# microsoft/M3P

Measured on AMD Instinct MI355X. Metric: pre-train samples/sec (whole node), 12L/768d seq=128+36, higher is better.
Workload: dtype bf16; 1 GPU; cfg2: 12L/768d/12h, 36 regions + 128 tokens, V=250002, 19 MLM targets/seq + ITM BCE, dropout 0.10, adam_inverse_sqrt + clip 5; per_gpu_batch=256, global_batch=256, seq_len=164, parallelism=dp1, prewarm_steps=36

## Files before the change

include/m3p_hip.h:

```cpp
#ifndef M3P_HIP_H
#define M3P_HIP_H

#include <stddef.h>
#include <stdint.h>

#ifdef __cplusplus
extern "C" {
#endif

#define M3P_API __attribute__((visibility("default")))

#define M3P_OK 0
#define M3P_EINVAL (-1)
#define M3P_ENOTIMPL (-2)
#define M3P_ENOMEM (-3)

M3P_API const char* m3p_version(void);


enum {
  M3P_EPI_NONE = 0,
  M3P_EPI_BIAS = 1,
  M3P_EPI_BIAS_GELU = 2,
  M3P_EPI_BIAS_DROP_RES = 3,
// ... 44 lines not shown
                                    int M, int N, int K, float alpha, void* stream);
M3P_API int m3p_gemm_nn_streamk_f32(const void* A, int lda, const void* W, int ldw, int k_valid, float* C,
                                    int ldc, int M, int N, int K, float alpha, void* stream);
M3P_API int m3p_gemm_nn_w4_f32(const void* A, int lda, const void* W, int ldw, float* C, int ldc, int M, int N, int K, float alpha,
                               void* workspace, size_t workspace_bytes, void* stream);

M3P_API size_t m3p_gemm_wgrad_workspace_bytes(void);
M3P_API int m3p_gemm_wgrad_bf16(const void* dY, int lddy, const void* X, int ldx, float* dW, int lddw,
                                int M, int N, int K, float alpha, void* workspace, size_t workspace_bytes,
                                void* stream);
M3P_API int m3p_gemm_wgrad_store_bf16(const void* dY, int lddy, const void* X, int ldx, float* dW, int lddw, int M, int N, int K,
                                      float alpha, void* workspace, size_t workspace_bytes, void* stream);
M3P_API int m3p_gemm_wgrad_pair_bf16(const void* dYa, int lddya, const void* Xa, int ldxa, float* dWa, int lddwa, int Na, int Ka,
                                     const void* dYb, int lddyb, const void* Xb, int ldxb, float* dWb, int lddwb, int Nb, int Kb,
                                     int M, float alpha, void* workspace, size_t workspace_bytes, void* stream);


M3P_API int m3p_layernorm_fwd(const void* x, const float* gamma, const float* beta, const uint8_t* rowmask,
                              void* y, float* mean, float* rstd, int rows, int d, float eps, void* stream);

M3P_API int m3p_layernorm_bwd(const void* dy_a, const void* dy_b, const void* x, const float* gamma,
                              const float* mean, const float* rstd, const uint8_t* rowmask,
                              void* dx, void* dx_drop, float* dgamma, float* dbeta, float* dbias_drop,
                              int rows, int d, uint32_t seed, uint32_t thresh24, float inv_keep, void* stream);
M3P_API int m3p_layernorm_bwd_rows(const void* dy_a, const void* dy_b, const void* x, const float* gamma,
                                   const float* mean, const float* rstd, const uint8_t* rowmask,
                                   void* dx, void* dx_drop, float* dgamma, float* dbeta, float* dbias_drop,
                                   int rows, int d, uint32_t seed, uint32_t thresh24, float inv_keep,
                                   const int32_t* rng_rows, void* stream);

// ... 178 lines not shown
```

m3p_amd/csrc/gemm.hip:

```cpp
#include <mutex>
#include <type_traits>
#include "common.hpp"
#include "../../include/m3p_hip.h"
#include <hip/amd_detail/amd_hip_unsafe_atomics.h>

static int g_variant = 1;
extern "C" void m3p_debug_set_variant(int v) { g_variant = (v == 2 || v == 6) ? v : 1; }

namespace {

constexpr int BK = 64;
constexpr int ROWB = BK * 2;

template <int EPI>
__device__ __forceinline__ void epilogue_store(const M3PEpilogue& ep, bf16* __restrict__ C, int ldc,
                                               int M, int N, int m, int n, f32x4 acc, f32x4& csum) {
  if (m >= M || n >= N) return;
  const bool full = (n + 3 < N);
  float v[4] = {acc[0], acc[1], acc[2], acc[3]};
  const float alpha = (ep.alpha == 0.f) ? 1.f : ep.alpha;
  if (EPI == M3P_EPI_NONE || EPI == M3P_EPI_BIAS || EPI == M3P_EPI_RES) {
#pragma unroll
    for (int r = 0; r < 4; ++r) v[r] *= alpha;
  }
// ... 1660 lines not shown
        read_a(Q0{}, nxt * STAGE, fa0);
        F8_LGKM0();
      }
    }
  }
  if ((EPI == M3P_EPI_DGELU || EPI == M3P_EPI_MUL) && ep.colsum && csum_nw >= 0) flush_csum();
#undef F8_LGKM0
}


struct WgCursor {
  int c, t, mt, len;
};
struct WgradProblem {
  const bf16* dY; const bf16* X; float* dW;
  int lddy, ldx, lddw, tiles_i, tiles_j;
};

template <bool W_KN>
__global__ __launch_bounds__(512)
void gemm_nt_streamk_kernel(const bf16* __restrict__ A, int lda, const bf16* __restrict__ W, int ldw,
                            float* __restrict__ Cf, int ldc, int M, int N, int K, float alpha,
                            int tiles_m, int tiles_n, int CHUNK, int k_valid) {
  constexpr int BM = 256, BN = 128, NWAVES = 8;
  constexpr int A_BYTES = BM * ROWB, B_BYTES = BN * ROWB, STAGE = A_BYTES + B_BYTES;
  extern __shared__ __attribute__((aligned(16))) char smem[];
  const int tid = threadIdx.x, lane = tid & 63;
  const int wid = __builtin_amdgcn_readfirstlane(tid >> 6);
  const int ntile = tiles_m * tiles_n;
  const int nk = K / BK;
  const long long total_all = (long long)ntile * nk;
// ... 932 lines not shown
#pragma unroll
  for (int a = 0; a < 4; ++a)
#pragma unroll
    for (int b = 0; b < 4; ++b) {
      const int j = j0 + wj * 64 + b * 16 + ft;
#pragma unroll
      for (int r = 0; r < 4; ++r) {
        const int i = i0 + wi * 64 + a * 16 + fg * 4 + r;
        if (i < N && j < K) unsafeAtomicAdd(dW + (size_t)i * lddw + j, alpha * acc[a][b][r]);
      }
    }
}

template <bool YROWS>
__global__ __launch_bounds__(256)
void gemm_wgrad_w4_kernel(const bf16* __restrict__ dY_a, int lddy_a, const bf16* __restrict__ X_a, int ldx_a,
                          float* __restrict__ dW_a, int lddw_a, int M, int N, int K, float alpha,
                          int tiles_i, int tiles_j_a, int WR_CHUNK, float* __restrict__ ws, int* __restrict__ ws_tile,
                          int overwrite, WgradProblem pb) {
  const bf16* dY = dY_a;
  const bf16* X = X_a;
  float* dW = dW_a;
  int lddy = lddy_a, ldx = ldx_a, lddw = lddw_a, tiles_j = tiles_j_a;
  int tile_id0 = 0;
  constexpr int TI = 256, TJ = 256, KT = 64;
  constexpr int ROWB = 512;
  constexpr int Y_BYTES = KT * ROWB, STAGE = 2 * Y_BYTES;
  extern __shared__ __attribute__((aligned(16))) char smem[];
  const int tid = threadIdx.x, lane = tid & 63;
  const int wid = __builtin_amdgcn_readfirstlane(tid >> 6);
  const int ntile_a = tiles_i * tiles_j_a;
  const int ntile = ntile_a + pb.tiles_i * pb.tiles_j;
  const int nmt = M / KT;
  const long long total_all = (long long)ntile * nmt;
  const int nwg = gridDim.x;
  const int per_xcd = nwg >> 3;
  const int slot = (blockIdx.x & 7) * per_xcd + (blockIdx.x >> 3);
  const bool rr = (WR_CHUNK == 0);
  if (ws && tid == 0) ws_tile[slot] = -1;
  int total, seg_tile, seg_m0, seg_len;
  if (rr) {
    const int my_tiles = (ntile > slot) ? (ntile - slot + nwg - 1) / nwg : 0;
    if (my_tiles == 0) return;
    total = my_tiles * nmt;
    seg_tile = slot; seg_m0 = 0; seg_len = nmt;
  } else {
    const int C = max(nwg / ntile, 1);
    if (slot >= C * ntile) return;
    const int c = slot / ntile;
    seg_tile = slot - c * ntile;
    if (seg_tile >= ntile_a) {
      dY = pb.dY; X = pb.X; dW = pb.dW; lddy = pb.lddy; ldx = pb.ldx; lddw = pb.lddw; tiles_j = pb.tiles_j;
      seg_tile -= ntile_a;
      tile_id0 = ntile_a;
    }
    seg_m0 = (int)((long long)c * nmt / C);
    seg_len = (int)((long long)(c + 1) * nmt / C) - seg_m0;
    total = seg_len;
    if (total <= 0) return;
  }
  (void)total_all;
  auto locate = [&](int) {
    WgCursor cu;
    cu.c = 0; cu.t = seg_tile; cu.mt = 0; cu.len = seg_len;
    return cu;
  };
  auto advance = [&](WgCursor& cu) {
    if (++cu.mt == cu.len) { cu.mt = 0; cu.t += nwg; }
  };
// ... 260 lines not shown
#pragma unroll
  for (int c = 0; c < 8; ++c) { yf0[c] = yfrag(c); xf0[c] = frag(xl[c], xh[c]); }

  WgCursor cc = locate(g0);
  bool first = true;
  int n_seg = 0;
  auto kstep = [&](auto stage_c, int step) {
    if (first) wktile(std::true_type{}, stage_c);
    else wktile(std::false_type{}, stage_c);
    first = false;

    const bool last_of_tile = (cc.mt + 1 == cc.len) || (step + 1 == total);
    if (last_of_tile) {
      asm volatile("s_nop 15\n\ts_nop 15" ::: "memory");
      const int ti = cc.t / tiles_j, tj = cc.t - ti * tiles_j;
      float* dbase = dW + (size_t)(ti * TI + wi * 128 + fg * 4) * lddw + tj * TJ + wj * 128 + ft;
      const bool to_ws = (ws != nullptr) && !rr && n_seg == 0 && (step + 1 == total);
      if (to_ws) {
        asm volatile("s_waitcnt vmcnt(0)" ::: "memory");
        __builtin_amdgcn_s_barrier();
        asm volatile("" ::: "memory");
      }
#pragma nounroll
      for (int bb = 0; bb < 8; ++bb) {
        const int b = to_ws ? bb : ((bb + slot) & 7);
        float v[32];
#define WG_RD8(B)                                                                                   \
  _Pragma("unroll") for (int q = 0; q < 32; ++q) v[q] = 0.f;                                        \
  asm volatile("v_accvgpr_read_b32 %0, a[(" #B ")*32+0]\n\tv_accvgpr_read_b32 %1, a[(" #B ")*32+1]\n\t"   \
               "v_accvgpr_read_b32 %2, a[(" #B ")*32+2]\n\tv_accvgpr_read_b32 %3, a[(" #B ")*32+3]\n\t"   \
               "v_accvgpr_read_b32 %4, a[(" #B ")*32+4]\n\tv_accvgpr_read_b32 %5, a[(" #B ")*32+5]\n\t"   \
               "v_accvgpr_read_b32 %6, a[(" #B ")*32+6]\n\tv_accvgpr_read_b32 %7, a[(" #B ")*32+7]"       \
// ... 20 lines not shown
          case 3: { WG_RD8(3); } break;
          case 4: { WG_RD8(4); } break;
          case 5: { WG_RD8(5); } break;
          case 6: { WG_RD8(6); } break;
          default: { WG_RD8(7); } break;
        }
#undef WG_RD8
        if (to_ws) {
          float* lw = reinterpret_cast<float*>(smem) + wid * (128 * 36) + (fg * 4) * 36 + (b & 1) * 16 + ft;
#pragma unroll
          for (int a = 0; a < 8; ++a)
#pragma unroll
            for (int r = 0; r < 4; ++r) lw[(a * 16 + r) * 36] = v[a * 4 + r];
          if (b & 1) {
            const float* lr = reinterpret_cast<const float*>(smem) + wid * (128 * 36) + (lane >> 3) * 36 + (lane & 7) * 4;
            float* wrow = ws + (size_t)slot * (TI * TJ + 272) + (size_t)(wi * 128 + (lane >> 3)) * TJ + wj * 128 + (b >> 1) * 32 + (lane & 7) * 4;
#pragma unroll
            for (int it = 0; it < 16; ++it)
              *reinterpret_cast<f32x4*>(wrow + it * 8 * TJ) = *reinterpret_cast<const f32x4*>(lr + it * 8 * 36);
          }
        } else {
          float* dcol = dbase + b * 16;
#pragma unroll
          for (int a = 0; a < 8; ++a)
#pragma unroll
            for (int r = 0; r < 4; ++r)
              if (overwrite) dcol[(size_t)(a * 16 + r) * lddw] = alpha * v[a * 4 + r];
              else unsafeAtomicAdd(dcol + (size_t)(a * 16 + r) * lddw, alpha * v[a * 4 + r]);
        }
      }
      if (to_ws && tid == 0) ws_tile[slot] = tile_id0 + cc.t;
      ++n_seg;
      first = true;
    }
    advance(cc);
  };
  for (int step = 0; step < total; step += 2) {
    kstep(std::integral_constant<int, 0>{}, step);
    if (step + 1 < total) kstep(std::integral_constant<int, 1>{}, step + 1);
  }
  asm volatile("s_waitcnt vmcnt(0)" ::: "memory");
#undef WG_LDB
#undef WG_TR2
#undef WG_YRD
#undef WG_LGKM0
#undef WG_ACC
#undef WG_M
#undef WG_L
}

__global__ __launch_bounds__(256)
void wgrad_reduce_kernel(const float* __restrict__ ws, const int* __restrict__ ws_tile, int nslots,
                         float* __restrict__ dW, int lddw, int tiles_j, float alpha, int ntile_a, WgradProblem pb) {
  const int t = blockIdx.y, rg = blockIdx.x;
  int tl = t;
  if (t >= ntile_a) { tl = t - ntile_a; dW = pb.dW; lddw = pb.lddw; tiles_j = pb.tiles_j; }
  const int ti = tl / tiles_j, tj = tl - ti * tiles_j;
  const int col = (threadIdx.x & 63) * 4, row0 = rg * 16 + (threadIdx.x >> 6) * 4;
  f32x4 acc[4];
#pragma unroll
  for (int r = 0; r < 4; ++r) acc[r] = f32x4{0.f, 0.f, 0.f, 0.f};
  bool any = false;
  const int ntile = gridDim.y;
  for (int s = t; s < nslots; s += ntile) {
    if (ws_tile[s] != t) continue;
    any = true;
    const float* p = ws + (size_t)s * (65536 + 272) + row0 * 256 + col;
#pragma unroll
    for (int r = 0; r < 4; ++r) acc[r] += *reinterpret_cast<const f32x4*>(p + r * 256);
  }
  if (!any) return;
// ... 325 lines not shown
  g_tq_slots = counters ? n_slots : 0;
  g_tq_next = 0;
  g_tq_bound = false;
  return M3P_OK;
}

size_t m3p_gemm_wgrad_workspace_bytes(void) {
  const size_t grid = (size_t)hw_cus();
  return grid * (65536 + 272) * sizeof(float) + grid * sizeof(int);
}

static bool wgrad_w4_ok(int M, int N, int K, int lddy, int ldx, const void* dY, const void* X) {
  return (M % 64) == 0 && M >= 4096 && (N % 256) == 0 && (K % 256) == 0 &&
         (lddy % 8) == 0 && (ldx % 8) == 0 && !((uintptr_t)dY & 15) && !((uintptr_t)X & 15);
}
extern "C++" {
template <bool YROWS = false>
static int launch_wgrad_w4(const void* dY, int lddy, const void* X, int ldx, float* dW, int lddw, int M, int N, int K,
                           float alpha, void* workspace, size_t workspace_bytes, void* stream, const WgradProblem* pb_in,
                           bool store = false) {
  const int ti = N / 256, tj = K / 256;
  WgradProblem pb = {};
  if (pb_in) pb = *pb_in;
  const int ntile = ti * tj + pb.tiles_i * pb.tiles_j;
  const size_t lds = 2 * 65536;
  static bool attr_set_w = false;
  if (!attr_set_w) {
    hipError_t e = hipFuncSetAttribute((const void*)gemm_wgrad_w4_kernel<YROWS>, hipFuncAttributeMaxDynamicSharedMemorySize, (int)lds);
    if (e != hipSuccess) return (int)e;
    attr_set_w = true;
  }
  const int grid = num_cus();
  const int nmt = M / 64;
  long long share = ((long long)ntile * nmt + grid - 1) / grid;
  int chunk = (int)(share < nmt ? (share < 1 ? 1 : share) : nmt);
  if ((long long)ntile >= 4LL * grid) chunk = 0;
  if (pb_in && chunk == 0) return M3P_EINVAL;
  if (store && chunk != 0) return M3P_ENOTIMPL;
  float* ws = nullptr;
  if (workspace && workspace_bytes >= m3p_gemm_wgrad_workspace_bytes() && (((uintptr_t)workspace & 15) == 0) && chunk != 0 &&
      (lddw % 4) == 0 && (((uintptr_t)dW & 15) == 0) && (!pb_in || ((pb.lddw % 4) == 0 && (((uintptr_t)pb.dW & 15) == 0))))
    ws = (float*)workspace;
  int* ws_tile = ws ? (int*)(ws + (size_t)grid * (65536 + 272)) : nullptr;
  hipLaunchKernelGGL(gemm_wgrad_w4_kernel<YROWS>, dim3(grid), dim3(256), lds, (hipStream_t)stream, (const bf16*)dY, lddy,
                     (const bf16*)X, ldx, dW, lddw, M, N, K, alpha, ti, tj, chunk, ws, ws_tile, store ? 1 : 0, pb);
  M3P_CHECK_LAUNCH();
  if (ws) {
    hipLaunchKernelGGL(wgrad_reduce_kernel, dim3(16, ntile), dim3(256), 0, (hipStream_t)stream, (const float*)ws,
                       (const int*)ws_tile, grid, dW, lddw, tj, alpha, ti * tj, pb);
    M3P_CHECK_LAUNCH();
  }
  return M3P_OK;
}
}

static int wgrad_plan(int M, int N, int K, bool aligned) {
  if (aligned && (M % 64) == 0 && M >= 4096 && (N % 256) == 0 && (K % 256) == 0 && (N / 256) * (K / 256) >= 9)
    return ((long long)(N / 256) * (K / 256) >= 4LL * num_cus()) ? M3P_KERN_WGRAD_W4_TILES : M3P_KERN_WGRAD_W4_CHUNKS;
  if ((M % BK) == 0 && M >= 4096) return M3P_KERN_WGRAD_RING;
  return M3P_KERN_WGRAD_128;
}

int m3p_gemm_nt_plan(int M, int N, int K, int epilogue) {
  if (M <= 0 || N <= 0 || K <= 0 || (K % BK) != 0 || epilogue < 0 || epilogue > M3P_EPI_BIAS_LSE) return M3P_EINVAL;
  int queue = 0;
  const int plan = nt_plan(epilogue, M, N, K, &queue);
  return (plan == M3P_KERN_NT_W8 && queue) ? M3P_KERN_NT_W8_QUEUE : plan;
}

int m3p_gemm_wgrad_plan(int M, int N, int K) {
  if (M <= 0 || N <= 0 || K <= 0) return M3P_EINVAL;
  return wgrad_plan(M, N, K, true);
}

int m3p_gemm_nn_w4_f32(const void* A, int lda, const void* W, int ldw, float* C, int ldc, int M, int N, int K, float alpha,
                       void* workspace, size_t workspace_bytes, void* stream) {
  if (M <= 0 || N <= 0 || K <= 0 || !A || !W || !C) return M3P_EINVAL;
  if ((K % 64) || K < 4096 || (M % 256) || (N % 256) || (lda % 8) || (ldw % 8) || lda < K || ldw < N || ldc < N ||
      ((uintptr_t)A & 15) || ((uintptr_t)W & 15))
    return M3P_ENOTIMPL;
  return launch_wgrad_w4<true>(A, lda, W, ldw, C, ldc, K, M, N, alpha, workspace, workspace_bytes, stream, nullptr);
}

int m3p_gemm_wgrad_pair_bf16(const void* dYa, int lddya, const void* Xa, int ldxa, float* dWa, int lddwa, int Na, int Ka,
                             const void* dYb, int lddyb, const void* Xb, int ldxb, float* dWb, int lddwb, int Nb, int Kb,
                             int M, float alpha, void* workspace, size_t workspace_bytes, void* stream) {
  if (M <= 0 || Na <= 0 || Ka <= 0 || Nb <= 0 || Kb <= 0) return M3P_EINVAL;
  const bool pair = wgrad_w4_ok(M, Na, Ka, lddya, ldxa, dYa, Xa) && wgrad_w4_ok(M, Nb, Kb, lddyb, ldxb, dYb, Xb) &&
                    workspace && workspace_bytes >= m3p_gemm_wgrad_workspace_bytes() && (((uintptr_t)workspace & 15) == 0) &&
                    (lddwa % 4) == 0 && (lddwb % 4) == 0 && (((uintptr_t)dWa | (uintptr_t)dWb) & 15) == 0 &&
                    lddwa >= Ka && lddwb >= Kb &&
                    (long long)((Na / 256) * (Ka / 256) + (Nb / 256) * (Kb / 256)) * 2 <= num_cus();
  if (!pair) {
    int rc = m3p_gemm_wgrad_bf16(dYa, lddya, Xa, ldxa, dWa, lddwa, M, Na, Ka, alpha, workspace, workspace_bytes, stream);
    if (rc != M3P_OK) return rc;
    return m3p_gemm_wgrad_bf16(dYb, lddyb, Xb, ldxb, dWb, lddwb, M, Nb, Kb, alpha, workspace, workspace_bytes, stream);
  }
  if (lddya < Na || ldxa < Ka || lddyb < Nb || ldxb < Kb) return M3P_EINVAL;
  WgradProblem pb = {(const bf16*)dYb, (const bf16*)Xb, dWb, lddyb, ldxb, lddwb, Nb / 256, Kb / 256};
  return launch_wgrad_w4<>(dYa, lddya, Xa, ldxa, dWa, lddwa, M, Na, Ka, alpha, workspace, workspace_bytes, stream, &pb);
}

int m3p_gemm_wgrad_store_bf16(const void* dY, int lddy, const void* X, int ldx, float* dW, int lddw, int M, int N, int K,
                              float alpha, void* workspace, size_t workspace_bytes, void* stream) {
  if (M <= 0 || N <= 0 || K <= 0 || (lddy % 8) != 0 || (ldx % 8) != 0 || !dW || lddw < K) return M3P_EINVAL;
  if (lddy < N || ldx < K || ((uintptr_t)dY & 15) || ((uintptr_t)X & 15)) return M3P_EINVAL;
  if (!wgrad_w4_ok(M, N, K, lddy, ldx, dY, X)) return M3P_ENOTIMPL;
  return launch_wgrad_w4<>(dY, lddy, X, ldx, dW, lddw, M, N, K, alpha, workspace, workspace_bytes, stream, nullptr, true);
}

int m3p_gemm_wgrad_bf16(const void* dY, int lddy, const void* X, int ldx, float* dW, int lddw, int M, int N, int K,
                        float alpha, void* workspace, size_t workspace_bytes, void* stream) {
  if (M <= 0 || N <= 0 || K <= 0 || (lddy % 8) != 0 || (ldx % 8) != 0 || !dW || lddw < K) return M3P_EINVAL;
  if (lddy < ((N + 7) / 8) * 8 || ldx < ((K + 7) / 8) * 8) return M3P_EINVAL;
  if (((uintptr_t)dY & 15) || ((uintptr_t)X & 15)) return M3P_EINVAL;
  const int plan = wgrad_plan(M, N, K, wgrad_w4_ok(M, N, K, lddy, ldx, dY, X));
  if (plan == M3P_KERN_WGRAD_W4_CHUNKS || plan == M3P_KERN_WGRAD_W4_TILES) {
    return launch_wgrad_w4<>(dY, lddy, X, ldx, dW, lddw, M, N, K, alpha, workspace, workspace_bytes, stream, nullptr);
  }
  if (plan == M3P_KERN_WGRAD_RING) {
    const int ti = (N + WR_I - 1) / WR_I, tj = (K + WR_J - 1) / WR_J;
    const size_t lds = 3 * WR_STAGE;
    static bool attr_set_r = false;
    if (!attr_set_r) {
      hipError_t e = hipFuncSetAttribute((const void*)gemm_wgrad_ring_kernel, hipFuncAttributeMaxDynamicSharedMemorySize, (int)lds);
      if (e != hipSuccess) return (int)e;
      attr_set_r = true;
    }
    const int grid = num_cus();
    const int nmt = M / BK;
    long long share = ((long long)ti * tj * nmt + grid - 1) / grid;
    int chunk = (int)(share < nmt ? (share < 1 ? 1 : share) : nmt);
    if ((long long)ti * tj >= 4LL * grid) chunk = 0;
// ... 28 lines not shown
```

m3p_amd/functional.py:

```python
import math
import os
from collections import OrderedDict

import torch

from . import lib as L
from . import fp8 as fp8mod
from . import ops
from . import rng

BF16 = torch.bfloat16
ALIGN = 64
BUCKET_ALIGN = 64 * 8


def _round_up(n, a):
    return (n + a - 1) // a * a


_VOCAB_FULL_TILES = os.environ.get('M3P_VOCAB_FULL_TILES', '1') != '0'
_GELU_GRAD_IN_FWD = os.environ.get('M3P_GELU_GRAD_IN_FWD', '0') != '0'
_GELU_BYTE_GRAD = int(os.environ.get('M3P_GELU_BYTE_GRAD', '2'))
_CE_FUSED_LSE = os.environ.get('M3P_CE_FUSED_LSE', '1') != '0'
_VOCAB_DGRAD_W4 = os.environ.get('M3P_VOCAB_DGRAD_W4', '1') != '0'
# ... 645 lines not shown
        sunk = ctx.sink.take()
        if dout is None and sunk is None:
            if hook is not None:
                hook.encoder_backward_end()
            return (None,) * N_ENC_ARGS
        if dout is None:
            dh_ = sunk
        else:
            dh_ = dout.contiguous()
            if dh_.dtype != BF16:
                dh_ = dh_.to(BF16)
            if sunk is not None:
                dh_ = dh_ + sunk.view_as(dh_)
        last = hook.encoder_backward_begin() if hook is not None else True
        st8 = model.fp8_state() if model.fp8 else None

        def dgrad(g, i, gsite, wsite, wt16, epi, pre8=None, **kw):
            if st8 is None or wsite not in fp8mod.BWD_SITES:
                return ops.gemm_nt(g, wt16, epi, **kw)
            g8, dgs = pre8 if pre8 is not None else st8.quant(g, i, gsite)
            _, wt8, dws = st8.weights[(i, wsite)]
            return ops.gemm_nt_fp8(g8, wt8, epi, a_is_bf8=True, descale_a=dgs, descale_b=dws, **kw)

        for i in reversed(range(nL)):
            a, f = 'attentions.%d.' % i, 'ffns.%d.' % i
            (h_in, qkv, ctxt, lse, pre1, mean1, rstd1, x1, u, hact, pre2, mean2, rstd2, ctx_c, mask_i) = saved_layers[i]
            saved_layers[i] = None
            compact = rows_c is not None and i == nL - 1
            rr = {}
            if compact:
                rr = dict(rng_rows=rows_c.idx)
                dh_ = ops.gather_rows(dh_.view(M, d), rows_c.idx, rows_c.n, d)
            dpre2, dY2 = ops.layernorm_bwd(dh_, None, pre2, ar.p('layer_norm2.%d.weight' % i), mean2, rstd2, mask_i,
                                           ar.g('layer_norm2.%d.weight' % i), ar.g('layer_norm2.%d.bias' % i),
                                           dbias_drop=ar.g(f + 'lin2.bias'), want_drop=p_drop > 0,
                                           seed=seed('ffn', i), p_drop=p_drop, **rr)
            if dY2 is None:
                dY2 = dpre2
            ops.gemm_wgrad(dY2, hact, ar.g(f + 'lin2.weight'))
            du8 = None
            if ctx.u_holds_grad == 'q':
                o8 = {}
                if st8 is not None and 'w1' in fp8mod.BWD_SITES:
                    kd = st8.index(i, 'du')
                    if st8.seen[kd]:
                        o8 = dict(out8=torch.empty((M, 4 * d), dtype=torch.uint8, device=dY2.device), scale8=st8.scale[kd:kd + 1],
                                  amax8=st8.amax[kd:kd + 1], out8_bf8=True)
                dU = ops.gemm_nt(dY2, ar.wt[('lin2', i)], L.EPI_MULQ, aux=u, colsum=ar.g(f + 'lin1.bias'), **o8)
                if o8:
                    du8 = (o8['out8'], st8.descale[kd:kd + 1])
                elif st8 is not None and 'w1' in fp8mod.BWD_SITES:
                    st8._first_use(dU, kd)
            else:
                dU = dgrad(dY2, i, 'dy2', 'w2', ar.wt[('lin2', i)], L.EPI_MUL if ctx.u_holds_grad else L.EPI_DGELU, aux=u,
                           colsum=ar.g(f + 'lin1.bias'))
            del hact, u, pre2
            ops.gemm_wgrad(dU, x1, ar.g(f + 'lin1.weight'))
            dx1 = dgrad(dU, i, 'du', 'w1', ar.wt[('lin1', i)], L.EPI_RES, aux=dpre2, pre8=du8)
            del dU, dpre2, dY2
            dpre1, dAO = ops.layernorm_bwd(dx1, None, pre1, ar.p('layer_norm1.%d.weight' % i), mean1, rstd1, None,
                                           ar.g('layer_norm1.%d.weight' % i), ar.g('layer_norm1.%d.bias' % i),
                                           dbias_drop=ar.g(a + 'out_lin.bias'), want_drop=p_drop > 0,
                                           seed=seed('attn_out', i), p_drop=p_drop, **rr)
            if dAO is None:
                dAO = dpre1
            dctx = dgrad(dAO, i, 'dao', 'wout', ar.wt[('out', i)], L.EPI_NONE)
            if compact:
                ops.gemm_wgrad(dAO, ctx_c, ar.g(a + 'out_lin.weight'))
                dctx = ops.place_rows(dctx, rows_c.inv, M, 0)
                dpre1 = ops.place_rows(dpre1, rows_c.inv, M, 0)
            dqkv = ops.attn_bwd(qkv, totlen, ctxt, dctx, lse[0], B, S, H, dh, dbias_qkv=ar.qkv_bias(i, grad=True),
                                seed=seed('attn_p', i), p_drop=p_attn, keepmask=lse[1])
            if compact:
                ops.gemm_wgrad(dqkv, h_in, ar.qkv_wgrad(i))
            else:
                ops.gemm_wgrad_pair(dqkv, h_in, ar.qkv_wgrad(i), dAO, ctxt, ar.g(a + 'out_lin.weight'))
            dh_ = dgrad(dqkv, i, 'dqkv', 'wqkv', ar.wt[('qkv', i)], L.EPI_RES, aux=dpre1)
            del dqkv, dctx, dAO, dpre1, dx1
            ar.touch_layer(i)
            if hook is not None:
                hook.layer_done(i, last)
        if ctx.h0_mode is not None:
            if hook is not None:
                hook.embed_done(last, ids=None, rows=None, n_max=ctx.tok_rows_max)
            return (None,) * 14 + (dh_.to(ctx.h0_mode), None, None)
        want_dximg, has_text_embed = ctx.input_grads
        langs, positions = ctx.langs, ctx.positions
        tok_rows = None
        if has_text_embed or langs is not None or positions is not None or (hook is not None and hook.active):
            tok_rows = torch.empty((T * B, d), dtype=BF16, device=dh_.device)
        grads = dict(
            d_g_emb=ar.g('layer_norm_emb.weight'), d_be_emb=ar.g('layer_norm_emb.bias'),
            d_pos=ar.g('position_embeddings.weight'), d_emb=ar.g('embeddings.weight'),
            d_g_img=ar.g('image_embeddings.LayerNorm.weight'), d_be_img=ar.g('image_embeddings.LayerNorm.bias'),
            d_b_img=ar.g('image_embeddings.image_embeddings.bias'),
            d_b_loc=ar.g('image_embeddings.image_location_embeddings.bias'),
# ... 709 lines not shown
```

m3p_amd/lib.py:

```python
import ctypes as C
import os

import torch

_HERE = os.path.dirname(os.path.abspath(__file__))
LIB_PATH = os.environ.get('M3P_HIP_LIB') or os.path.join(_HERE, 'libm3p_hip.so')

EPI_NONE, EPI_BIAS, EPI_BIAS_GELU, EPI_BIAS_DROP_RES, EPI_RES, EPI_DGELU, EPI_MUL, EPI_MULQ, EPI_BIAS_GELUQ, EPI_BIAS_LSE = range(10)
KERN_NT_SKINNY, KERN_NT_W8, KERN_NT_W8_QUEUE, KERN_NT_W4, KERN_NT_RING, KERN_NT_128 = range(1, 7)
KERN_WGRAD_W4_CHUNKS, KERN_WGRAD_W4_TILES, KERN_WGRAD_RING, KERN_WGRAD_128 = range(10, 14)


class M3PError(RuntimeError):
    pass


class Epilogue(C.Structure):
    _fields_ = [
        ('bias', C.c_void_p), ('aux', C.c_void_p), ('out2', C.c_void_p), ('colsum', C.c_void_p),
        ('ld_aux', C.c_int32), ('ld_out2', C.c_int32), ('scale_cols', C.c_int32), ('scale', C.c_float),
        ('alpha', C.c_float), ('seed', C.c_uint32), ('thresh24', C.c_uint32), ('inv_keep', C.c_float),
        ('descale_a', C.c_void_p), ('descale_b', C.c_void_p),
        ('out8', C.c_void_p), ('scale8', C.c_void_p), ('amax8', C.c_void_p), ('ld_out8', C.c_int32), ('out8_bf8', C.c_int32),
        ('rng_rows', C.c_void_p),
        ('row_ref', C.c_void_p),
    ]


_p, _i, _f, _u32 = C.c_void_p, C.c_int, C.c_float, C.c_uint32

SIGNATURES = {
    'm3p_version': (C.c_char_p, []),
    'm3p_gemm_nt_bf16': (_i, [_p, _i, _p, _i, _p, _i, _i, _i, _i, _i, C.POINTER(Epilogue), _p]),
    'm3p_gemm_nt_fp8': (_i, [_p, _i, _i, _p, _i, _p, _i, _i, _i, _i, _i, C.POINTER(Epilogue), _p]),
    'm3p_quant_fp8': (_i, [_p, _i, _p, _i, _i, _i, _p, _p, _i, _p]),
    'm3p_quant_fp8_batch': (_i, [_p, _i, _i, _p]),
    'm3p_gemm_nt_streamk_f32': (_i, [_p, _i, _p, _i, _p, _i, _i, _i, _i, _f, _p]),
    'm3p_gemm_nn_streamk_f32': (_i, [_p, _i, _p, _i, _i, _p, _i, _i, _i, _i, _f, _p]),
    'm3p_gemm_nn_w4_f32': (_i, [_p, _i, _p, _i, _p, _i, _i, _i, _i, _f, _p, C.c_size_t, _p]),
    'm3p_gemm_wgrad_workspace_bytes': (C.c_size_t, []),
    'm3p_gemm_wgrad_bf16': (_i, [_p, _i, _p, _i, _p, _i, _i, _i, _i, _f, _p, C.c_size_t, _p]),
    'm3p_gemm_wgrad_store_bf16': (_i, [_p, _i, _p, _i, _p, _i, _i, _i, _i, _f, _p, C.c_size_t, _p]),
    'm3p_gemm_wgrad_pair_bf16': (_i, [_p, _i, _p, _i, _p, _i, _i, _i, _p, _i, _p, _i, _p, _i, _i, _i, _i, _f, _p, C.c_size_t, _p]),
    'm3p_layernorm_fwd': (_i, [_p, _p, _p, _p, _p, _p, _p, _i, _i, _f, _p]),
    'm3p_layernorm_bwd': (_i, [_p, _p, _p, _p, _p, _p, _p, _p, _p, _p, _p, _p, _i, _i, _u32, _u32, _f, _p]),
    'm3p_layernorm_bwd_rows': (_i, [_p, _p, _p, _p, _p, _p, _p, _p, _p, _p, _p, _p, _i, _i, _u32, _u32, _f, _p, _p]),
    'm3p_attn_fwd': (_i, [_p, _p, _p, _p, _p, _i, _i, _i, _i, _u32, _u32, _f, _p]),
    'm3p_attn_bwd': (_i, [_p, _p, _p, _p, _p, _p, _p, _p, _i, _i, _i, _i, _f, _u32, _u32, _f, _p]),
    'm3p_attn_query_fwd': (_i, [_p, _i, _p, C.c_longlong, _i, _p, _p, _i, _i, _i, _i, _i, _i, _i, _p]),
    'm3p_attn_rows_fwd': (_i, [_p, _i, _p, C.c_longlong, _i, _p, _p, _p, _i, _i, _i, _i, _i, _i, _i, _u32, _u32, _f, _p]),
    'm3p_attn_rows_bwd': (_i, [_p, _i, _p, C.c_longlong, _i, _p, _p, _p, _p, _i, _p, _i, _i, _i, _i, _i, _i, _i, _f, _u32, _u32, _f, _p]),
    'm3p_attn_causal_fwd': (_i, [_p, _i, _p, _p, _i, _i, _i, _i, _u32, _u32, _f, _p]),
    'm3p_attn_causal_bwd': (_i, [_p, _i, _p, _p, _p, _i, _i, _i, _i, _i, _f, _u32, _u32, _f, _p]),
    'm3p_cast_f32_bf16': (_i, [_p, _p, C.c_longlong, _p]),
    'm3p_embed_assemble_fwd': (_i, [_p] * 19 + [_i, _i, _i, _i, _u32, _u32, _u32, _f, _p, _p]),
    'm3p_embed_image_rows_fwd': (_i, [_p] * 10 + [_i, _i, _i, _u32, _u32, _f, _p]),
    'm3p_embed_assemble_bwd': (_i, [_p] * 24 + [_i, _i, _i, _i, _i, _u32, _u32, _u32, _f, _i, _p]),
    'm3p_dropout_rows': (_i, [_p, _i, _p, _i, _p, _i, _i, _i, _u32, _u32, _u32, _u32, _f, _p]),
# ... 95 lines not shown
```

m3p_amd/ops.py:

```python
import ctypes as C
import os

import torch

from . import lib as L

BF16 = torch.bfloat16
_DEBUG_CHECKS = os.environ.get('M3P_DEBUG_CHECKS') == '1'

PROFILE = None
_EPI_NAMES = ['gemm_nt/none', 'gemm_nt/bias', 'gemm_nt/bias_gelu', 'gemm_nt/bias_drop_res', 'gemm_nt/res',
              'gemm_nt/dgelu', 'gemm_nt/mul', 'gemm_nt/mulq', 'gemm_nt/bias_geluq', 'gemm_nt/bias_lse']


PROFILE_ONLY = None


def _prof_begin(key=None):
    if PROFILE is None or (PROFILE_ONLY is not None and key != PROFILE_ONLY):
        return None
    e = torch.cuda.Event(enable_timing=True)
    e.record()
    return e

# ... 200 lines not shown
    _chk_bf16(dy_a, x_a, dy_b, x_b)
    assert dw_a.dtype == torch.float32 and dw_b.dtype == torch.float32 and dw_a.stride(-1) == 1 and dw_b.stride(-1) == 1
    M = dy_a.shape[0]
    assert x_a.shape[0] == M and dy_b.shape[0] == M and x_b.shape[0] == M
    Na, Ka, Nb, Kb = dy_a.shape[1], x_a.shape[1], dy_b.shape[1], x_b.shape[1]
    assert dw_a.shape[0] >= Na and dw_a.shape[1] >= Ka and dw_b.shape[0] >= Nb and dw_b.shape[1] >= Kb
    e0 = _prof_begin(('gemm_wgrad_pair', M, Na + Nb, Ka))
    ws = _wgrad_workspace(dy_a.device)
    rc = L.load().m3p_gemm_wgrad_pair_bf16(dy_a.data_ptr(), dy_a.stride(0), x_a.data_ptr(), x_a.stride(0), dw_a.data_ptr(), dw_a.stride(0),
                                           Na, Ka, dy_b.data_ptr(), dy_b.stride(0), x_b.data_ptr(), x_b.stride(0), dw_b.data_ptr(),
                                           dw_b.stride(0), Nb, Kb, M, alpha, ws.data_ptr(), ws.numel(), L.stream())
    L.check(rc, 'm3p_gemm_wgrad_pair_bf16')
    _prof_end(e0, ('gemm_wgrad_pair', M, Na + Nb, Ka))


def layernorm_fwd(x, gamma, beta, rowmask=None, eps=1e-12):
    _chk_bf16(x)
    rows, d = x.shape
    assert x.is_contiguous()
    y = torch.empty_like(x)
    mean = torch.empty(rows, dtype=torch.float32, device=x.device)
    rstd = torch.empty(rows, dtype=torch.float32, device=x.device)
    rc = L.load().m3p_layernorm_fwd(x.data_ptr(), gamma.data_ptr(), beta.data_ptr(), L.ptr(rowmask), y.data_ptr(),
                                    mean.data_ptr(), rstd.data_ptr(), rows, d, eps, L.stream())
    L.check(rc, 'm3p_layernorm_fwd')
    return y, mean, rstd


def layernorm_bwd(dy_a, dy_b, x, gamma, mean, rstd, rowmask, dgamma, dbeta, dbias_drop=None,
                  want_drop=False, seed=0, p_drop=0.0, rng_rows=None):
# ... 617 lines not shown
```

Baseline: 8262 sequences/s.

## Group weight-gradient GEMMs across layers into single multi-problem launches

Adds a grouped wgrad entry point that takes up to 16 weight-gradient problems and runs them in one persistent kernel with a tile table. On the Python side, encoder backward now defers per-layer wgrad GEMMs and batches them until they fill the CUs. When each tile gets exactly one workgroup, a direct mode does a read-add-write into dW and skips the workspace and reduce kernel. The aim is fewer small launches and better CU occupancy for the 768-wide wgrads. In exchange, deferral keeps activations and gradients alive longer, and the direct read-modify-write relies on no other workgroup writing the same tile.

```diff
diff --git a/include/m3p_hip.h b/include/m3p_hip.h
--- a/include/m3p_hip.h
+++ b/include/m3p_hip.h
@@ -82,6 +82,16 @@
 M3P_API int m3p_gemm_wgrad_pair_bf16(const void* dYa, int lddya, const void* Xa, int ldxa, float* dWa, int lddwa, int Na, int Ka,
                                      const void* dYb, int lddyb, const void* Xb, int ldxb, float* dWb, int lddwb, int Nb, int Kb,
                                      int M, float alpha, void* workspace, size_t workspace_bytes, void* stream);
+#define M3P_WGRAD_GROUP_MAX 16
+typedef struct {
+  const void* dY;
+  const void* X;
+  float* dW;
+  int lddy, ldx, lddw;
+  int N, K;
+} m3p_wgrad_item;
+M3P_API int m3p_gemm_wgrad_group_bf16(const m3p_wgrad_item* items, int n_items, int M, float alpha, void* workspace,
+                                      size_t workspace_bytes, void* stream);
 
 
 M3P_API int m3p_layernorm_fwd(const void* x, const float* gamma, const float* beta, const uint8_t* rowmask,
diff --git a/m3p_amd/csrc/gemm.hip b/m3p_amd/csrc/gemm.hip
--- a/m3p_amd/csrc/gemm.hip
+++ b/m3p_amd/csrc/gemm.hip
@@ -1698,7 +1698,11 @@
 };
 struct WgradProblem {
   const bf16* dY; const bf16* X; float* dW;
-  int lddy, ldx, lddw, tiles_i, tiles_j;
+  int lddy, ldx, lddw, tiles_i, tiles_j, tile0;
+};
+struct WgradTable {
+  int n, ntile;
+  WgradProblem p[M3P_WGRAD_GROUP_MAX];
 };
 
 template <bool W_KN>
@@ -2661,26 +2665,23 @@
 
 template <bool YROWS>
 __global__ __launch_bounds__(256)
-void gemm_wgrad_w4_kernel(const bf16* __restrict__ dY_a, int lddy_a, const bf16* __restrict__ X_a, int ldx_a,
-                          float* __restrict__ dW_a, int lddw_a, int M, int N, int K, float alpha,
-                          int tiles_i, int tiles_j_a, int WR_CHUNK, float* __restrict__ ws, int* __restrict__ ws_tile,
-                          int overwrite, WgradProblem pb) {
-  const bf16* dY = dY_a;
-  const bf16* X = X_a;
-  float* dW = dW_a;
-  int lddy = lddy_a, ldx = ldx_a, lddw = lddw_a, tiles_j = tiles_j_a;
-  int tile_id0 = 0;
+void gemm_wgrad_w4_kernel(int M, float alpha, int WR_CHUNK, float* __restrict__ ws, int flags, WgradTable tab) {
+  const bf16* dY = tab.p[0].dY;
+  const bf16* X = tab.p[0].X;
+  int lddy = tab.p[0].lddy, ldx = tab.p[0].ldx, tiles_j = tab.p[0].tiles_j;
+  int pi = 0;
   constexpr int TI = 256, TJ = 256, KT = 64;
   constexpr int ROWB = 512;
   constexpr int Y_BYTES = KT * ROWB, STAGE = 2 * Y_BYTES;
   extern __shared__ __attribute__((aligned(16))) char smem[];
   const int tid = threadIdx.x, lane = tid & 63;
   const int wid = __builtin_amdgcn_readfirstlane(tid >> 6);
-  const int ntile_a = tiles_i * tiles_j_a;
-  const int ntile = ntile_a + pb.tiles_i * pb.tiles_j;
+  const int ntile = tab.ntile;
   const int nmt = M / KT;
   const long long total_all = (long long)ntile * nmt;
   const int nwg = gridDim.x;
+  const bool overwrite = (flags & 1) != 0, direct = (flags & 2) != 0;
+  int* ws_tile = reinterpret_cast<int*>(ws + (size_t)nwg * (TI * TJ + 272));
   const int per_xcd = nwg >> 3;
   const int slot = (blockIdx.x & 7) * per_xcd + (blockIdx.x >> 3);
   const bool rr = (WR_CHUNK == 0);
@@ -2696,10 +2697,12 @@
     if (slot >= C * ntile) return;
     const int c = slot / ntile;
     seg_tile = slot - c * ntile;
-    if (seg_tile >= ntile_a) {
-      dY = pb.dY; X = pb.X; dW = pb.dW; lddy = pb.lddy; ldx = pb.ldx; lddw = pb.lddw; tiles_j = pb.tiles_j;
-      seg_tile -= ntile_a;
-      tile_id0 = ntile_a;
+#pragma nounroll
+    for (int q = 1; q < tab.n; ++q) pi = (seg_tile >= tab.p[q].tile0) ? q : pi;
+    if (pi != 0) {
+      const WgradProblem& pb = tab.p[pi];
+      dY = pb.dY; X = pb.X; lddy = pb.lddy; ldx = pb.ldx; tiles_j = pb.tiles_j;
+      seg_tile -= pb.tile0;
     }
     seg_m0 = (int)((long long)c * nmt / C);
     seg_len = (int)((long long)(c + 1) * nmt / C) - seg_m0;
@@ -2990,8 +2993,10 @@
     if (last_of_tile) {
       asm volatile("s_nop 15\n\ts_nop 15" ::: "memory");
       const int ti = cc.t / tiles_j, tj = cc.t - ti * tiles_j;
+      float* const dW = tab.p[pi].dW;
+      const int lddw = tab.p[pi].lddw, tile_id0 = tab.p[pi].tile0;
       float* dbase = dW + (size_t)(ti * TI + wi * 128 + fg * 4) * lddw + tj * TJ + wj * 128 + ft;
-      const bool to_ws = (ws != nullptr) && !rr && n_seg == 0 && (step + 1 == total);
+      const bool to_ws = (ws != nullptr || direct) && !rr && n_seg == 0 && (step + 1 == total);
       if (to_ws) {
         asm volatile("s_waitcnt vmcnt(0)" ::: "memory");
         __builtin_amdgcn_s_barrier();
@@ -3042,10 +3047,25 @@
             for (int r = 0; r < 4; ++r) lw[(a * 16 + r) * 36] = v[a * 4 + r];
           if (b & 1) {
             const float* lr = reinterpret_cast<const float*>(smem) + wid * (128 * 36) + (lane >> 3) * 36 + (lane & 7) * 4;
-            float* wrow = ws + (size_t)slot * (TI * TJ + 272) + (size_t)(wi * 128 + (lane >> 3)) * TJ + wj * 128 + (b >> 1) * 32 + (lane & 7) * 4;
-#pragma unroll
-            for (int it = 0; it < 16; ++it)
-              *reinterpret_cast<f32x4*>(wrow + it * 8 * TJ) = *reinterpret_cast<const f32x4*>(lr + it * 8 * 36);
+            if (direct) {
+              float* drow = dW + (size_t)(ti * TI + wi * 128 + (lane >> 3)) * lddw + tj * TJ + wj * 128 + (b >> 1) * 32 + (lane & 7) * 4;
+              const size_t dstep = (size_t)8 * lddw;
+#pragma unroll
+              for (int h = 0; h < 2; ++h) {
+                f32x4 old[8];
+#pragma unroll
+                for (int it = 0; it < 8; ++it) old[it] = *reinterpret_cast<const f32x4*>(drow + (h * 8 + it) * dstep);
+#pragma unroll
+                for (int it = 0; it < 8; ++it)
+                  *reinterpret_cast<f32x4*>(drow + (h * 8 + it) * dstep) =
+                      old[it] + alpha * *reinterpret_cast<const f32x4*>(lr + (h * 8 + it) * 8 * 36);
+              }
+            } else {
+              float* wrow = ws + (size_t)slot * (TI * TJ + 272) + (size_t)(wi * 128 + (lane >> 3)) * TJ + wj * 128 + (b >> 1) * 32 + (lane & 7) * 4;
+#pragma unroll
+              for (int it = 0; it < 16; ++it)
+                *reinterpret_cast<f32x4*>(wrow + it * 8 * TJ) = *reinterpret_cast<const f32x4*>(lr + it * 8 * 36);
+            }
           }
         } else {
           float* dcol = dbase + b * 16;
@@ -3057,7 +3077,7 @@
               else unsafeAtomicAdd(dcol + (size_t)(a * 16 + r) * lddw, alpha * v[a * 4 + r]);
         }
       }
-      if (to_ws && tid == 0) ws_tile[slot] = tile_id0 + cc.t;
+      if (to_ws && ws && tid == 0) ws_tile[slot] = tile_id0 + cc.t;
       ++n_seg;
       first = true;
     }
@@ -3079,10 +3099,12 @@
 
 __global__ __launch_bounds__(256)
 void wgrad_reduce_kernel(const float* __restrict__ ws, const int* __restrict__ ws_tile, int nslots,
-                         float* __restrict__ dW, int lddw, int tiles_j, float alpha, int ntile_a, WgradProblem pb) {
+                         float alpha, WgradTable tab) {
   const int t = blockIdx.y, rg = blockIdx.x;
-  int tl = t;
-  if (t >= ntile_a) { tl = t - ntile_a; dW = pb.dW; lddw = pb.lddw; tiles_j = pb.tiles_j; }
+  int pi = 0;
+  for (int q = 1; q < tab.n; ++q) pi = (t >= tab.p[q].tile0) ? q : pi;
+  float* dW = tab.p[pi].dW;
+  const int lddw = tab.p[pi].lddw, tiles_j = tab.p[pi].tiles_j, tl = t - tab.p[pi].tile0;
   const int ti = tl / tiles_j, tj = tl - ti * tiles_j;
   const int col = (threadIdx.x & 63) * 4, row0 = rg * 16 + (threadIdx.x >> 6) * 4;
   f32x4 acc[4];
@@ -3438,15 +3460,24 @@
   return (M % 64) == 0 && M >= 4096 && (N % 256) == 0 && (K % 256) == 0 &&
          (lddy % 8) == 0 && (ldx % 8) == 0 && !((uintptr_t)dY & 15) && !((uintptr_t)X & 15);
 }
+static void wgrad_table_add(WgradTable& tab, const void* dY, int lddy, const void* X, int ldx, float* dW, int lddw, int N, int K) {
+  tab.p[tab.n] = WgradProblem{(const bf16*)dY, (const bf16*)X, dW, lddy, ldx, lddw, N / 256, K / 256, tab.ntile};
+  tab.ntile += (N / 256) * (K / 256);
+  ++tab.n;
+}
+static bool wgrad_table_dw16(const WgradTable& tab) {
+  for (int q = 0; q < tab.n; ++q)
+    if ((tab.p[q].lddw % 4) != 0 || ((uintptr_t)tab.p[q].dW & 15) != 0) return false;
+  return true;
+}
+static bool wgrad_ws_ok(const void* workspace, size_t workspace_bytes) {
+  return workspace && workspace_bytes >= m3p_gemm_wgrad_workspace_bytes() && (((uintptr_t)workspace & 15) == 0);
+}
 extern "C++" {
 template <bool YROWS = false>
-static int launch_wgrad_w4(const void* dY, int lddy, const void* X, int ldx, float* dW, int lddw, int M, int N, int K,
-                           float alpha, void* workspace, size_t workspace_bytes, void* stream, const WgradProblem* pb_in,
-                           bool store = false) {
-  const int ti = N / 256, tj = K / 256;
-  WgradProblem pb = {};
-  if (pb_in) pb = *pb_in;
-  const int ntile = ti * tj + pb.tiles_i * pb.tiles_j;
+static int launch_wgrad_w4(const WgradTable& tab, int M, float alpha, void* workspace, size_t workspace_bytes, void* stream,
+                           bool store = false, bool need16 = false) {
+  const int ntile = tab.ntile;
   const size_t lds = 2 * 65536;
   static bool attr_set_w = false;
   if (!attr_set_w) {
@@ -3459,22 +3490,30 @@
   long long share = ((long long)ntile * nmt + grid - 1) / grid;
   int chunk = (int)(share < nmt ? (share < 1 ? 1 : share) : nmt);
   if ((long long)ntile >= 4LL * grid) chunk = 0;
-  if (pb_in && chunk == 0) return M3P_EINVAL;
+  if (tab.n > 1 && chunk == 0) return M3P_EINVAL;
   if (store && chunk != 0) return M3P_ENOTIMPL;
+  const bool dw16 = wgrad_table_dw16(tab);
+  const int direct = (chunk != 0 && ntile <= grid && grid / ntile == 1 && dw16) ? 1 : 0;
   float* ws = nullptr;
-  if (workspace && workspace_bytes >= m3p_gemm_wgrad_workspace_bytes() && (((uintptr_t)workspace & 15) == 0) && chunk != 0 &&
-      (lddw % 4) == 0 && (((uintptr_t)dW & 15) == 0) && (!pb_in || ((pb.lddw % 4) == 0 && (((uintptr_t)pb.dW & 15) == 0))))
-    ws = (float*)workspace;
+  if (!direct && wgrad_ws_ok(workspace, workspace_bytes) && chunk != 0 && dw16) ws = (float*)workspace;
+  if (need16 && !direct && !ws) return M3P_ENOTIMPL;
   int* ws_tile = ws ? (int*)(ws + (size_t)grid * (65536 + 272)) : nullptr;
-  hipLaunchKernelGGL(gemm_wgrad_w4_kernel<YROWS>, dim3(grid), dim3(256), lds, (hipStream_t)stream, (const bf16*)dY, lddy,
-                     (const bf16*)X, ldx, dW, lddw, M, N, K, alpha, ti, tj, chunk, ws, ws_tile, store ? 1 : 0, pb);
+  hipLaunchKernelGGL(gemm_wgrad_w4_kernel<YROWS>, dim3(grid), dim3(256), lds, (hipStream_t)stream, M, alpha, chunk, ws,
+                     (store ? 1 : 0) | (direct ? 2 : 0), tab);
   M3P_CHECK_LAUNCH();
   if (ws) {
     hipLaunchKernelGGL(wgrad_reduce_kernel, dim3(16, ntile), dim3(256), 0, (hipStream_t)stream, (const float*)ws,
-                       (const int*)ws_tile, grid, dW, lddw, tj, alpha, ti * tj, pb);
+                       (const int*)ws_tile, grid, alpha, tab);
     M3P_CHECK_LAUNCH();
   }
   return M3P_OK;
+}
+template <bool YROWS = false>
+static int launch_wgrad_w4(const void* dY, int lddy, const void* X, int ldx, float* dW, int lddw, int M, int N, int K,
+                           float alpha, void* workspace, size_t workspace_bytes, void* stream, bool store = false) {
+  WgradTable tab = {};
+  wgrad_table_add(tab, dY, lddy, X, ldx, dW, lddw, N, K);
+  return launch_wgrad_w4<YROWS>(tab, M, alpha, workspace, workspace_bytes, stream, store);
 }
 }
 
@@ -3503,7 +3542,7 @@
   if ((K % 64) || K < 4096 || (M % 256) || (N % 256) || (lda % 8) || (ldw % 8) || lda < K || ldw < N || ldc < N ||
       ((uintptr_t)A & 15) || ((uintptr_t)W & 15))
     return M3P_ENOTIMPL;
-  return launch_wgrad_w4<true>(A, lda, W, ldw, C, ldc, K, M, N, alpha, workspace, workspace_bytes, stream, nullptr);
+  return launch_wgrad_w4<true>(A, lda, W, ldw, C, ldc, K, M, N, alpha, workspace, workspace_bytes, stream);
 }
 
 int m3p_gemm_wgrad_pair_bf16(const void* dYa, int lddya, const void* Xa, int ldxa, float* dWa, int lddwa, int Na, int Ka,
@@ -3511,7 +3550,7 @@
                              int M, float alpha, void* workspace, size_t workspace_bytes, void* stream) {
   if (M <= 0 || Na <= 0 || Ka <= 0 || Nb <= 0 || Kb <= 0) return M3P_EINVAL;
   const bool pair = wgrad_w4_ok(M, Na, Ka, lddya, ldxa, dYa, Xa) && wgrad_w4_ok(M, Nb, Kb, lddyb, ldxb, dYb, Xb) &&
-                    workspace && workspace_bytes >= m3p_gemm_wgrad_workspace_bytes() && (((uintptr_t)workspace & 15) == 0) &&
+                    wgrad_ws_ok(workspace, workspace_bytes) &&
                     (lddwa % 4) == 0 && (lddwb % 4) == 0 && (((uintptr_t)dWa | (uintptr_t)dWb) & 15) == 0 &&
                     lddwa >= Ka && lddwb >= Kb &&
                     (long long)((Na / 256) * (Ka / 256) + (Nb / 256) * (Kb / 256)) * 2 <= num_cus();
@@ -3521,8 +3560,24 @@
     return m3p_gemm_wgrad_bf16(dYb, lddyb, Xb, ldxb, dWb, lddwb, M, Nb, Kb, alpha, workspace, workspace_bytes, stream);
   }
   if (lddya < Na || ldxa < Ka || lddyb < Nb || ldxb < Kb) return M3P_EINVAL;
-  WgradProblem pb = {(const bf16*)dYb, (const bf16*)Xb, dWb, lddyb, ldxb, lddwb, Nb / 256, Kb / 256};
-  return launch_wgrad_w4<>(dYa, lddya, Xa, ldxa, dWa, lddwa, M, Na, Ka, alpha, workspace, workspace_bytes, stream, &pb);
+  const m3p_wgrad_item items[2] = {{dYa, Xa, dWa, lddya, ldxa, lddwa, Na, Ka}, {dYb, Xb, dWb, lddyb, ldxb, lddwb, Nb, Kb}};
+  return m3p_gemm_wgrad_group_bf16(items, 2, M, alpha, workspace, workspace_bytes, stream);
+}
+
+int m3p_gemm_wgrad_group_bf16(const m3p_wgrad_item* items, int n_items, int M, float alpha, void* workspace,
+                              size_t workspace_bytes, void* stream) {
+  if (!items || n_items <= 0 || M <= 0) return M3P_EINVAL;
+  if (n_items > M3P_WGRAD_GROUP_MAX) return M3P_ENOTIMPL;
+  WgradTable tab = {};
+  for (int q = 0; q < n_items; ++q) {
+    const m3p_wgrad_item& it = items[q];
+    if (it.N <= 0 || it.K <= 0 || !it.dY || !it.X || !it.dW) return M3P_EINVAL;
+    if (!wgrad_w4_ok(M, it.N, it.K, it.lddy, it.ldx, it.dY, it.X)) return M3P_ENOTIMPL;
+    if (it.lddy < it.N || it.ldx < it.K || it.lddw < it.K) return M3P_EINVAL;
+    wgrad_table_add(tab, it.dY, it.lddy, it.X, it.ldx, it.dW, it.lddw, it.N, it.K);
+  }
+  if (tab.ntile > num_cus() || !wgrad_table_dw16(tab)) return M3P_ENOTIMPL;
+  return launch_wgrad_w4<>(tab, M, alpha, workspace, workspace_bytes, stream, false, true);
 }
 
 int m3p_gemm_wgrad_store_bf16(const void* dY, int lddy, const void* X, int ldx, float* dW, int lddw, int M, int N, int K,
@@ -3530,7 +3585,7 @@
   if (M <= 0 || N <= 0 || K <= 0 || (lddy % 8) != 0 || (ldx % 8) != 0 || !dW || lddw < K) return M3P_EINVAL;
   if (lddy < N || ldx < K || ((uintptr_t)dY & 15) || ((uintptr_t)X & 15)) return M3P_EINVAL;
   if (!wgrad_w4_ok(M, N, K, lddy, ldx, dY, X)) return M3P_ENOTIMPL;
-  return launch_wgrad_w4<>(dY, lddy, X, ldx, dW, lddw, M, N, K, alpha, workspace, workspace_bytes, stream, nullptr, true);
+  return launch_wgrad_w4<>(dY, lddy, X, ldx, dW, lddw, M, N, K, alpha, workspace, workspace_bytes, stream, true);
 }
 
 int m3p_gemm_wgrad_bf16(const void* dY, int lddy, const void* X, int ldx, float* dW, int lddw, int M, int N, int K,
@@ -3540,7 +3595,7 @@
   if (((uintptr_t)dY & 15) || ((uintptr_t)X & 15)) return M3P_EINVAL;
   const int plan = wgrad_plan(M, N, K, wgrad_w4_ok(M, N, K, lddy, ldx, dY, X));
   if (plan == M3P_KERN_WGRAD_W4_CHUNKS || plan == M3P_KERN_WGRAD_W4_TILES) {
-    return launch_wgrad_w4<>(dY, lddy, X, ldx, dW, lddw, M, N, K, alpha, workspace, workspace_bytes, stream, nullptr);
+    return launch_wgrad_w4<>(dY, lddy, X, ldx, dW, lddw, M, N, K, alpha, workspace, workspace_bytes, stream);
   }
   if (plan == M3P_KERN_WGRAD_RING) {
     const int ti = (N + WR_I - 1) / WR_I, tj = (K + WR_J - 1) / WR_J;
diff --git a/m3p_amd/functional.py b/m3p_amd/functional.py
--- a/m3p_amd/functional.py
+++ b/m3p_amd/functional.py
@@ -683,6 +683,7 @@
                 dh_ = dh_ + sunk.view_as(dh_)
         last = hook.encoder_backward_begin() if hook is not None else True
         st8 = model.fp8_state() if model.fp8 else None
+        wg = ops.WgradCollector(M, enabled=model.ddp_hook is None)
 
         def dgrad(g, i, gsite, wsite, wt16, epi, pre8=None, **kw):
             if st8 is None or wsite not in fp8mod.BWD_SITES:
@@ -706,7 +707,7 @@
                                            seed=seed('ffn', i), p_drop=p_drop, **rr)
             if dY2 is None:
                 dY2 = dpre2
-            ops.gemm_wgrad(dY2, hact, ar.g(f + 'lin2.weight'))
+            wg.add(dY2, hact, ar.g(f + 'lin2.weight'))
             du8 = None
             if ctx.u_holds_grad == 'q':
                 o8 = {}
@@ -724,7 +725,7 @@
                 dU = dgrad(dY2, i, 'dy2', 'w2', ar.wt[('lin2', i)], L.EPI_MUL if ctx.u_holds_grad else L.EPI_DGELU, aux=u,
                            colsum=ar.g(f + 'lin1.bias'))
             del hact, u, pre2
-            ops.gemm_wgrad(dU, x1, ar.g(f + 'lin1.weight'))
+            wg.add(dU, x1, ar.g(f + 'lin1.weight'))
             dx1 = dgrad(dU, i, 'du', 'w1', ar.wt[('lin1', i)], L.EPI_RES, aux=dpre2, pre8=du8)
             del dU, dpre2, dY2
             dpre1, dAO = ops.layernorm_bwd(dx1, None, pre1, ar.p('layer_norm1.%d.weight' % i), mean1, rstd1, None,
@@ -735,20 +736,22 @@
                 dAO = dpre1
             dctx = dgrad(dAO, i, 'dao', 'wout', ar.wt[('out', i)], L.EPI_NONE)
             if compact:
-                ops.gemm_wgrad(dAO, ctx_c, ar.g(a + 'out_lin.weight'))
+                wg.add(dAO, ctx_c, ar.g(a + 'out_lin.weight'))
                 dctx = ops.place_rows(dctx, rows_c.inv, M, 0)
                 dpre1 = ops.place_rows(dpre1, rows_c.inv, M, 0)
             dqkv = ops.attn_bwd(qkv, totlen, ctxt, dctx, lse[0], B, S, H, dh, dbias_qkv=ar.qkv_bias(i, grad=True),
                                 seed=seed('attn_p', i), p_drop=p_attn, keepmask=lse[1])
             if compact:
-                ops.gemm_wgrad(dqkv, h_in, ar.qkv_wgrad(i))
+                wg.add(dqkv, h_in, ar.qkv_wgrad(i))
             else:
-                ops.gemm_wgrad_pair(dqkv, h_in, ar.qkv_wgrad(i), dAO, ctxt, ar.g(a + 'out_lin.weight'))
+                wg.add_pair(dqkv, h_in, ar.qkv_wgrad(i), dAO, ctxt, ar.g(a + 'out_lin.weight'))
             dh_ = dgrad(dqkv, i, 'dqkv', 'wqkv', ar.wt[('qkv', i)], L.EPI_RES, aux=dpre1)
             del dqkv, dctx, dAO, dpre1, dx1
             ar.touch_layer(i)
             if hook is not None:
                 hook.layer_done(i, last)
+        wg.flush()
+        assert not wg.items
         if ctx.h0_mode is not None:
             if hook is not None:
                 hook.embed_done(last, ids=None, rows=None, n_max=ctx.tok_rows_max)
diff --git a/m3p_amd/lib.py b/m3p_amd/lib.py
--- a/m3p_amd/lib.py
+++ b/m3p_amd/lib.py
@@ -27,6 +27,13 @@
     ]
 
 
+class WgradItem(C.Structure):
+    _fields_ = [('dY', C.c_void_p), ('X', C.c_void_p), ('dW', C.c_void_p), ('lddy', C.c_int32), ('ldx', C.c_int32),
+                ('lddw', C.c_int32), ('N', C.c_int32), ('K', C.c_int32)]
+
+
+WGRAD_GROUP_MAX = 16
+
 _p, _i, _f, _u32 = C.c_void_p, C.c_int, C.c_float, C.c_uint32
 
 SIGNATURES = {
@@ -42,6 +49,7 @@
     'm3p_gemm_wgrad_bf16': (_i, [_p, _i, _p, _i, _p, _i, _i, _i, _i, _f, _p, C.c_size_t, _p]),
     'm3p_gemm_wgrad_store_bf16': (_i, [_p, _i, _p, _i, _p, _i, _i, _i, _i, _f, _p, C.c_size_t, _p]),
     'm3p_gemm_wgrad_pair_bf16': (_i, [_p, _i, _p, _i, _p, _i, _i, _i, _p, _i, _p, _i, _p, _i, _i, _i, _i, _f, _p, C.c_size_t, _p]),
+    'm3p_gemm_wgrad_group_bf16': (_i, [C.POINTER(WgradItem), _i, _i, _f, _p, C.c_size_t, _p]),
     'm3p_layernorm_fwd': (_i, [_p, _p, _p, _p, _p, _p, _p, _i, _i, _f, _p]),
     'm3p_layernorm_bwd': (_i, [_p, _p, _p, _p, _p, _p, _p, _p, _p, _p, _p, _p, _i, _i, _u32, _u32, _f, _p]),
     'm3p_layernorm_bwd_rows': (_i, [_p, _p, _p, _p, _p, _p, _p, _p, _p, _p, _p, _p, _i, _i, _u32, _u32, _f, _p, _p]),
diff --git a/m3p_amd/ops.py b/m3p_amd/ops.py
--- a/m3p_amd/ops.py
+++ b/m3p_amd/ops.py
@@ -238,6 +238,103 @@
     _prof_end(e0, ('gemm_wgrad_pair', M, Na + Nb, Ka))
 
 
+def wgrad_tiles(n, k):
+    return (n // 256) * (k // 256)
+
+
+def wgrad_groupable(m, n, k):
+    return m % 64 == 0 and m >= 4096 and n % 256 == 0 and k % 256 == 0 and wgrad_tiles(n, k) >= 9
+
+
+def plan_wgrad_groups(tiles, n_cus, min_frac=None, max_items=L.WGRAD_GROUP_MAX):
+    min_frac = WGRAD_GROUP_MIN_FRAC if min_frac is None else min_frac
+    groups, cur, cur_t, big = [], [], 0, []
+    for i, t in enumerate(tiles):
+        if t > n_cus:
+            big.append(i)
+            continue
+        if cur and (cur_t + t > n_cus or len(cur) == max_items):
+            groups.append(cur)
+            cur, cur_t = [], 0
+        cur.append(i)
+        cur_t += t
+    if cur and cur_t >= min_frac * n_cus:
+        groups.append(cur)
+        cur = []
+    return groups, sorted(big + cur)
+
+
+WGRAD_GROUP_MIN_FRAC = 0.75
+
+
+def gemm_wgrad_group(items, alpha=1.0):
+    M = items[0][0].shape[0]
+    arr = (L.WgradItem * len(items))()
+    ntile = 0
+    for q, (dy, x, dw) in enumerate(items):
+        _chk_bf16(dy, x)
+        assert dw.dtype == torch.float32 and dw.stride(-1) == 1 and dy.stride(1) == 1 and x.stride(1) == 1
+        N, K = dy.shape[1], x.shape[1]
+        assert dy.shape[0] == M and x.shape[0] == M and dw.shape[0] >= N and dw.shape[1] >= K
+        arr[q] = L.WgradItem(dy.data_ptr(), x.data_ptr(), dw.data_ptr(), dy.stride(0), x.stride(0), dw.stride(0), N, K)
+        ntile += wgrad_tiles(N, K)
+    key = ('gemm_wgrad_group', M, 256 * ntile, 256)
+    e0 = _prof_begin(key)
+    ws = _wgrad_workspace(items[0][0].device)
+    rc = L.load().m3p_gemm_wgrad_group_bf16(arr, len(items), M, alpha, ws.data_ptr(), ws.numel(), L.stream())
+    L.check(rc, 'm3p_gemm_wgrad_group_bf16')
+    _prof_end(e0, key)
+
+
+class WgradCollector:
+
+    def __init__(self, M, enabled=True):
+        self.M, self.enabled = M, enabled
+        self.items, self.tiles = [], 0
+        self.n_cus = L.num_cus()
+
+    def _takes(self, dy, x):
+        return self.enabled and dy.shape[0] == self.M and x.shape[0] == self.M and wgrad_groupable(self.M, dy.shape[1], x.shape[1]) \
+            and wgrad_tiles(dy.shape[1], x.shape[1]) <= self.n_cus
+
+    def add(self, dy, x, dw, _pair=False):
+        if not self._takes(dy, x):
+            gemm_wgrad(dy, x, dw)
+            return
+        t = wgrad_tiles(dy.shape[1], x.shape[1])
+        if self.items and (self.tiles + t > self.n_cus or len(self.items) == L.WGRAD_GROUP_MAX):
+            self._launch()
+        self.items.append((dy, x, dw, _pair))
+        self.tiles += t
+
+    def add_pair(self, dy_a, x_a, dw_a, dy_b, x_b, dw_b):
+        if not (self._takes(dy_a, x_a) and self._takes(dy_b, x_b)):
+            gemm_wgrad_pair(dy_a, x_a, dw_a, dy_b, x_b, dw_b)
+            return
+        self.add(dy_a, x_a, dw_a, _pair=True)
+        self.add(dy_b, x_b, dw_b)
+
+    def _launch(self):
+        items, self.items, self.tiles = self.items, [], 0
+        gemm_wgrad_group([it[:3] for it in items])
+
+    def flush(self):
+        if not self.items:
+            return
+        if self.tiles >= WGRAD_GROUP_MIN_FRAC * self.n_cus:
+            self._launch()
+            return
+        items, self.items, self.tiles = self.items, [], 0
+        q = 0
+        while q < len(items):
+            if items[q][3] and q + 1 < len(items):
+                gemm_wgrad_pair(*items[q][:3], *items[q + 1][:3])
+                q += 2
+            else:
+                gemm_wgrad(*items[q][:3])
+                q += 1
+
+
 def layernorm_fwd(x, gamma, beta, rowmask=None, eps=1e-12):
     _chk_bf16(x)
     rows, d = x.shape
```

Result: no change. 8279 sequences/s (median of 3 runs) (+0.2%).
